# BloodAxe/segmentation-networks-benchmark

Measured on AMD Instinct MI355X. Metric: images/sec/GPU (fwd+bwd) ZF_UNET 224x224 bs=32; 1/2/4/8-GPU scaling, higher is better.
Workload: dtype bf16; 1 GPU; ZF_UNET 224x224 bf16 bs=32/GPU, bce_dice, SGD lr 1e-3, Dropout2d 0.2, train step torch_train.py:180-190 (configs[1]); global_batch=32, parallelism=dp1

## Files before the change

### segmentation-networks-benchmark_amd/csrc/common.h

```cpp
#pragma once
#include <hip/hip_runtime.h>
#include <hip/hip_ext.h>
#include <limits.h>
#include <stdint.h>
#include <stdio.h>
#include <string.h>

#include "../../include/segnb_hip.h"

typedef __attribute__((ext_vector_type(8))) __bf16 bf16x8_t;
typedef __attribute__((ext_vector_type(16))) float f32x16_t;

struct bf16_t {
    unsigned short bits;
};

void segnb_set_error(const char* fmt, ...);

#define SEGNB_CHECK_ARG_AS(who, cond, msg)                           \
    do {                                                             \
        if (!(cond)) {                                               \
            segnb_set_error("%s: bad argument: %s", who, msg);       \
            return SEGNB_E_BADARG;                                   \
        }                                                            \
// ... 126 lines not shown
    const long long yb = segnb_nhwc_bytes((long long)g->N * g->Ho * g->Wo, bn->ld_y, g->Co, 2);
    if (!segnb_fits_desc(yb)) return false;
    a.bn_y = (const bf16_t*)bn->y;
    a.bn_y_bytes = (unsigned)yb;
    a.bn_ld = bn->ld_y;
    a.bn_coef = bn->coef;
    a.bn_sums = bn->sums;
    a.bn_act = bn->act;
    a.bn_slope = bn->slope;
    return true;
}
template <class Args>
__attribute__((always_inline)) inline void take_act_epilogue(Args& a, const segnb_act_epilogue* ep) {
    a.ep_act = ep != nullptr ? ep->act : -1;
    a.ep_coef = ep != nullptr ? ep->coef : nullptr;
    a.ep_slope = ep != nullptr ? ep->slope : 0.f;
}
int segnb_fprop_thin_try(segnb_try_outcome* did, const segnb_conv_geom* g, const void* in, const void* wpacked, void* out,
                         hipStream_t stream, const segnb_bn_reduce_epilogue* bn);
int segnb_fprop_thin_ok(const segnb_conv_geom* g);
int segnb_knob_fprop_upd();
int segnb_knob_fprop_drop();
int segnb_knob_fprop_mask();
int segnb_fprop_dma_actmask_ok(const segnb_conv_geom* g);
int segnb_fprop_roll_actmask_ok(const segnb_conv_geom* g);
int segnb_knob_fprop_mf16();
int segnb_knob_fprop_rw();
int segnb_knob_fprop_ksplit();
float* segnb_head_scratch(size_t bytes, hipStream_t stream);
void segnb_head_bwd_finish(const float* part, int gx, int gy, int K, int C, int CT, float* dw, float* db, hipStream_t stream);
int segnb_knob_pack_blocks();
int segnb_knob_fprop_roll();
int segnb_knob_wg_cu_pct();
int segnb_knob_conv_cus();
int segnb_fprop_dma_read_stamps(unsigned long long* host_dst);
int segnb_fprop_s1_try(segnb_try_outcome* did, const segnb_conv_geom* g, const void* in, const void* wpacked, const float* bias, int bias_n,
                       void* out, double* stats, hipStream_t stream, const float* drop = nullptr, int ld_drop = 0, int stats_ld = 0);
int segnb_fprop_dma_try(segnb_try_outcome* did, const segnb_conv_geom* g, const void* in, unsigned in_bytes, const void* wpacked,
                        unsigned w_bytes, const float* bias, int bias_n, void* out, double* stats,
                        hipStream_t stream, const segnb_act_epilogue* ep = nullptr, const segnb_upcat_src* uc = nullptr,
                        const segnb_bn_reduce_epilogue* bn = nullptr);
int segnb_fprop_rw_try(segnb_try_outcome* did, const segnb_conv_geom* g, const void* in, unsigned in_bytes, const void* wpacked,
                       unsigned w_bytes, const float* bias, int bias_n, void* out, double* stats,
                       hipStream_t stream, const segnb_bn_reduce_epilogue* bn = nullptr,
                       const segnb_act_epilogue* ep = nullptr, const segnb_upcat_src* uc = nullptr,
                       const segnb_upcat_src* upsum = nullptr);
// ... 190 lines not shown
```

### segmentation-networks-benchmark_amd/csrc/conv_igemm.hip

```cpp
#include <stdlib.h>

#include "device.h"

namespace {

constexpr int LDS_ROW = 144;
constexpr int NT = 256;

struct FpropArgs {
    segnb_conv_geom g = {};
    const void* in = nullptr;
    const void* w = nullptr;
    const float* bias = nullptr;
    int bias_n = 0;
    const float* ep_coef = nullptr;
    int ep_act = -1;
    float ep_slope = 0.f;
    void* out = nullptr;
    double* stats = nullptr;
    int M = 0, Ktot = 0, ksteps = 0, MT = 0, NTL = 0, GM = 0;
    unsigned in_bytes = 0, w_bytes = 0;
    const void* bn_y = nullptr;
    int bn_ld = 0;
    const float* bn_coef = nullptr;
// ... 1256 lines not shown
extern "C" int segnb_conv_wgrad_upcat(const segnb_conv_geom* g, int dtype, const void* in, const segnb_upcat_src* src,
                                      const void* dout, float* dwp, int nslab, segnb_stream_t stream) {
    SEGNB_PLAN_RECORD(segnb_conv_wgrad_upcat, g, dtype, in, src, dout, dwp, nslab, stream);
    const segnb_wgrad_target* tgt;
    if (int rc = take_wgrad_target(__func__, g, &tgt)) return rc;
    SEGNB_CHECK_ARG(in && src && src->u && dout && dwp, "NULL tensor");
    SEGNB_CHECK_ARG(upcat_geom_ok(g, dtype, src->Cu), "geometry not served (segnb_conv_upcat_ok)");
    SEGNB_CHECK_ARG(nslab == segnb_conv_wgrad_slabs(g, dtype), "nslab differs from segnb_conv_wgrad_slabs()");
    segnb_try_outcome did;
    if (int rc = segnb_wgrad_s1_try(&did, g, in, dout, dwp, nslab, (hipStream_t)stream, false, nullptr, src, tgt)) return rc;
    return finish_wgrad(__func__, did, g, dwp, nslab, tgt, false, (hipStream_t)stream);
}

static bool out_slice_fits(const segnb_conv_geom* g, int ld) {
    return segnb_fits_desc(segnb_nhwc_bytes((long long)g->N * g->Ho * g->Wo, ld, g->Co, 2));
}

static bool bnreduce_general(const segnb_conv_geom* g) { return g->Ci <= 24 && g->Co >= 32 && g->Co % 8 == 0; }

extern "C" int segnb_conv_fprop_bnreduce_ok(const segnb_conv_geom* g, int dtype) {
    if (g == nullptr || dtype != SEGNB_BF16 || check_geom(g) || !segnb_knob_bnreduce_fused()) return 0;
    if (!whole_output_3x3_s1(g) || g->Co % 8 != 0) return 0;
    if (bnreduce_general(g)) return 1;
    if (segnb_fprop_general_forced() || !segnb_knob_fprop_dma() || !segnb_knob_fprop_rw() || g->Wo < 12) return 0;
    for (int t = 0; t < 9; ++t)
        if (g->dh[t] < -1 || g->dh[t] > 1 || g->dw[t] < -1 || g->dw[t] > 1) return 0;
    if (g->Ci % 32 != 0 || g->Ci > 96 || g->Co > 64) return 0;
    if (g->Co > 32 && g->Ci > 32) return 0;
    return 1;
}

extern "C" int segnb_conv_fprop_bnreduce(const segnb_conv_geom* g, int dtype, const void* in, const void* wpacked,
                                         void* out, const segnb_bn_reduce_epilogue* ep, segnb_stream_t stream) {
    SEGNB_PLAN_RECORD(segnb_conv_fprop_bnreduce, g, dtype, in, wpacked, out, ep, stream);
    if (int rc = check_geom(g)) return rc;
    SEGNB_CHECK_ARG(in && wpacked && out && ep && ep->y && ep->sums, "NULL argument");
    SEGNB_CHECK_ARG(ep->ld_y >= g->Co && ep->ld_y % 8 == 0, "bad y stride");
    unsigned inb, wb;
    if (int rc = conv_extents(__func__, g, 2, g->Ci, &inb, &wb)) return rc;
    const hipStream_t st = (hipStream_t)stream;
    int rc = 0;
    segnb_try_outcome did;
    if (ep->coef == nullptr) {
        SEGNB_CHECK_ARG(segnb_conv_fprop_actmask_ok(g, dtype), "geometry not served by a fused kernel (segnb_conv_fprop_actmask_ok)");
        if (segnb_fprop_roll_actmask_ok(g))
            rc = segnb_fprop_roll_try(&did, g, in, inb, wpacked, wb, nullptr, 0, out, nullptr, st, ep);
        else
            rc = segnb_fprop_dma_try(&did, g, in, inb, wpacked, wb, nullptr, 0, out, nullptr, st, nullptr, nullptr, ep);
    } else {
        SEGNB_CHECK_ARG(segnb_conv_fprop_bnreduce_ok(g, dtype), "geometry not served by a fused kernel (segnb_conv_fprop_bnreduce_ok)");
        if (bnreduce_general(g)) {
            SEGNB_CHECK_ARG(ep->ld_y % 8 == 0 && out_slice_fits(g, ep->ld_y), "bad y");
            return conv_fprop_impl(g, dtype, in, wpacked, nullptr, 0, out, nullptr, stream, nullptr, ep);
        }
        if (g->Ci <= 96) {
            rc = segnb_fprop_roll_try(&did, g, in, inb, wpacked, wb, nullptr, 0, out, nullptr, st, ep);
            if (!rc && !did) rc = segnb_fprop_rw_try(&did, g, in, inb, wpacked, wb, nullptr, 0, out, nullptr, st, ep);
        } else {
            rc = segnb_fprop_dma_try(&did, g, in, inb, wpacked, wb, nullptr, 0, out, nullptr, st, nullptr, nullptr, ep);
        }
    }
    return finish_fprop(__func__, rc, did, SEGNB_E_BADARG, "the fused kernel refused the launch");
}

extern "C" int segnb_conv_fprop_bnapply_ok(const segnb_conv_geom* g, int dtype) {
    if (g == nullptr || dtype != SEGNB_BF16 || check_geom(g) || !segnb_knob_bnreduce_fused()) return 0;
    if (!whole_output_3x3_s1(g) || g->Co % 8 != 0 || g->Co <= 32) return 0;
    return bnreduce_general(g) ? 1 : 0;
}

extern "C" int segnb_conv_fprop_bnsums(const segnb_conv_geom* g, int dtype, const void* in, const void* wpacked,
                                       const segnb_bn_reduce_epilogue* ep, segnb_stream_t stream) {
    SEGNB_PLAN_RECORD(segnb_conv_fprop_bnsums, g, dtype, in, wpacked, ep, stream);
    if (int rc = check_geom(g)) return rc;
    SEGNB_CHECK_ARG(in && wpacked && ep && ep->y && ep->coef && ep->sums, "NULL argument");
    SEGNB_CHECK_ARG(segnb_conv_fprop_bnapply_ok(g, dtype), "geometry not served (segnb_conv_fprop_bnapply_ok)");
    SEGNB_CHECK_ARG(ep->ld_y >= g->Co && ep->ld_y % 8 == 0 && out_slice_fits(g, ep->ld_y), "bad y");
    return conv_fprop_impl(g, dtype, in, wpacked, nullptr, 0, nullptr, nullptr, stream, nullptr, ep, nullptr, 1);
// ... 132 lines not shown
```

### segmentation-networks-benchmark_amd/csrc/fprop_dma.hip

```cpp
#include "common.h"

#include "fprop_dma.h"
#include "tile_div.h"

#include <mutex>
#include <vector>

namespace {

struct WsArgs : FdArgs {
    TileDiv div_hw, div_w;
};

__device__ unsigned long long g_stamps[3 * 256 * 4];
#define FD_STAMP(role, step, k)                                                                      \
    do {                                                                                            \
        if (DBG && ((a.dbg & 32) || ((a.dbg & 64) && (role) == 0 && (k) == 0)) && blockIdx.x == 0 && lane == 0 &&  \
            (step) < 256)                                                                            \
            g_stamps[((role) * 256 + (step)) * 4 + (k)] = __builtin_amdgcn_s_memtime();             \
    } while (0)

template <int BN_, int R_, int WT_, int CW_M_, bool TALL_ = false, bool MF16_ = true, int NTAP_ = 9, int UP_ = 0>
struct WsCfg {
    static constexpr bool UPD_ = UP_ == 1;
// ... 39 lines not shown
    static constexpr int OFF_BIAS = OFF_PIX + 4 * BM * 4;
    static constexpr int OFF_SCALE = OFF_BIAS + BN * 4;
    static constexpr int OFF_TICKET = OFF_SCALE + BN * 4;
    static constexpr int SMEM = OFF_TICKET + 16;
    static constexpr int RED_BYTES = MT * 16 * 8;
    static_assert(WM % (MF16_ ? 16 : 32) == 0 && WN % (MF16_ ? 16 : 32) == 0 && WAVES_M * WAVES_N == NCW, "wave tiling");
    static_assert(BPIECES % NBW == 0 && NBW + NAW == NLW, "fetch wave roles");
    static_assert(MT % OC == 0 && MT >= 2 * BN && RPT <= 8 && BM <= MT && BM % (MT / OC) == 0, "store pass / statistics threads");
    static constexpr bool MASK_OK = MF16_ && !TALL_ && BM == 256 && CW_M_ == 4 && SMEM + 2048 <= 160 * 1024;
    static_assert(RED_BYTES <= OFF_STG, "statistics reduction scratch");
    static_assert(SMEM <= 160 * 1024, "LDS");
    static_assert(TM + TN <= 6, "fragment wait statement");
};

template <class C_>
struct WsEpi : C_ {
    static constexpr bool EPI = true;
};
template <class C, class = void>
struct ws_epi_of : std::false_type {};
template <class C>
struct ws_epi_of<C, std::enable_if_t<C::EPI>> : std::true_type {};

template <class C, bool DBG, bool EP = false, bool STATS = true, bool SPLITK = false, bool MASK = false>
__global__ __launch_bounds__(512) void conv_fprop_ws_kernel(const WsArgs a) {
    static_assert(!SPLITK || (!EP && !DBG && C::UP == 0 && C::NTAP == 9), "split K: plain 3 x 3 forward / data gradient");
    static_assert(!MASK || (STATS && !EP && !DBG && !SPLITK && C::MF16 && C::UP == 0 && C::NTAP == 9 && !C::TALL && C::BM == 256 &&
                            C::BN == 64 && C::WAVES_M == 4 && C::SMEM + 2048 <= 160 * 1024),
                  "activation mask: plain 3 x 3 data gradient, 16x16x32 form, 256 x 64 tiles, 2 KB of mask bytes behind the LDS layout");
    constexpr int BN = C::BN, R = C::R, WT = C::WT, BM = C::BM, TM = C::TM, TN = C::TN, XC = C::XC;
    constexpr int NT = C::NT, NB = C::NB, APW = C::APW, APS = C::APS, BPW = C::BPW, OC = C::OC, NLW = C::NLW;
    constexpr int OUT_ROW = C::OUT_ROW, NF = TM + TN;
    constexpr int NTAP = C::NTAP, KW = C::KW;
    constexpr int SM = NTAP & 3;
    constexpr bool EPI = ws_epi_of<C>::value;
    static_assert(!EPI || (C::MF16 && !SPLITK && !EP && C::UP == 0 && C::NTAP == 9), "store rows on peeled taps: 16x16x32 form, 3 x 3 window, whole-K tiles");

    extern __shared__ __attribute__((aligned(1024))) unsigned char smem[];
    int* sPix = reinterpret_cast<int*>(smem + C::OFF_PIX);
    float* sBias = reinterpret_cast<float*>(smem + C::OFF_BIAS);
    const unsigned lds0 = (unsigned)(size_t)smem;

    const int tid = threadIdx.x, lane = tid & 63, wave = __builtin_amdgcn_readfirstlane(tid >> 6);
    const int r = lane & 31, h = lane >> 5;
    const bool loader = wave >= C::NCW;
    const int lw = wave - C::NCW;
    const int wm = (wave & 3) / C::WAVES_N, wn = (wave & 3) % C::WAVES_N;

    int L_ = xcd_remap(blockIdx.x, gridDim.x);
    int ks_ = 0, nt_, gq_;
    if (C::TALL && a.ntmajor) {
        gq_ = L_ % a.GM;
        L_ /= a.GM;
        if constexpr (SPLITK) {
            ks_ = L_ % a.KS;
            L_ /= a.KS;
        }
        nt_ = L_;
    } else {
// ... 72 lines not shown
                        const int pa_ = 2 * c, pb_ = 2 * c + 1;
                        const int ta = (2 * (t >> 1) - (pa_ >> 1) + 1) * 4 + (2 * (t & 1) - (pa_ & 1) + 1);
                        const int tb = (2 * (t >> 1) - (pb_ >> 1) + 1) * 4 + (2 * (t & 1) - (pb_ & 1) + 1);
        #pragma unroll
                        for (int pb = 0; pb < BPW; ++pb) {
                            const unsigned off = (unsigned)(((b_sec >> pb & 1u) ? tb : ta) * 32) * 2u;
                            dma16(lds0 + C::OFF_B + stage * C::B_STAGE + ((lw & 1) * BPW + pb) * 1024, b_voff[pb] + off, rs_w, 0u);
                        }
                        return;
                    }
                    const int pl = c / a.NCHP, sl = c - pl * a.NCHP;
                    const int t16 = (2 * (t >> 1) - (pl >> 1) + 1) * 4 + (2 * (t & 1) - (pl & 1) + 1);
                    soff = (unsigned)(t16 * a.Ci + sl * 64) * 2u;
                } else if constexpr (C::UPF) {
                    soff = (unsigned)((3 - t) * a.Ci + c * 64) * 2u;
                } else {
                    soff = (unsigned)(t * a.Ci + (c + c_off) * 64) * 2u;
                }
        #pragma unroll
                for (int pb = 0; pb < BPW; ++pb)
                    dma16(lds0 + C::OFF_B + stage * C::B_STAGE + ((lw & 1) * BPW + pb) * 1024, b_voff[pb], rs_w, soff);
            };

            fetch_b(0, 0, 0);
            fetch_b(0, 1, 1);
            fetch_b(0, 2, 2);
            asm volatile("s_waitcnt vmcnt(0)" ::: "memory");
            lds_barrier();
            for (; it < a.IT; it += a.GM) {
                for (int c = 0; c < a.NCH; ++c, ++cg) {
                    const int cn = c + 1 == a.NCH ? 0 : c + 1;
                    static_for<NTAP>([&](auto t_c) {
                        constexpr int t = decltype(t_c)::value;
                        constexpr int tf = t + 3 < NTAP ? t + 3 : t + 3 - NTAP;
                        const int cf = t + 3 < NTAP ? c : cn;
                        if (lw == 0) FD_STAMP(1, cg * 9 + t, 0);
                        if (!(DBG && (a.dbg & 1))) fetch_b(cf, tf, (cg * SM + t + 3) & (NB - 1));
                        if (lw == 0) FD_STAMP(1, cg * 9 + t, 1);
                        asm volatile("s_waitcnt vmcnt(%0)" ::"n"(BPW) : "memory");
                        if (lw == 0) FD_STAMP(1, cg * 9 + t, 2);
                        raw_barrier();
                        if (lw == 0) FD_STAMP(1, cg * 9 + t, 3);
                    });
                }
            }
        } else {
            unsigned a_rel[APW], a_xy[APW], a_voff[C::NPL][APW];
            unsigned a_uoff[APW];
            constexpr bool VCAT = !C::UPD && !C::UPF && !C::TALL;
            static_assert(!VCAT || (R % 2 == 0 && WT % 2 == 0), "virtual concat: even tile origins");
            unsigned a_urel[VCAT ? APW : 1];
            unsigned a_sec = 0;
            static_assert(APW <= 32, "one bit per halo piece");
            const bool vcat = VCAT && a.u != nullptr;
        #pragma unroll
            for (int pa = 0; pa < APW; ++pa) {
                const int pix = ((lw & 1) + C::NAW * pa) * 8 + (lane >> 3);
                const int q = lane & 7;
                const int xr = pix / XC, xc = pix - xr * XC;
                const int key = C::XC % 2 == 0 ? xc : pix;
                a_rel[pa] = (unsigned)((xr * a.Wi + xc) * (C::UPD ? 2 : 1)) * (unsigned)a.ld_x * 2u +
                            (unsigned)((q ^ ((key >> 1) & 7)) * 16);
                if constexpr (C::UPD)
                    if (a.P32)
                        a_rel[pa] = (unsigned)((xr * a.Wi + xc) * 2) * (unsigned)a.ld_x * 2u + (unsigned)(((q ^ ((key >> 1) & 7)) & 3) * 16);
                a_xy[pa] = pix < C::NPIX ? (unsigned)xr | ((unsigned)xc << 16) : 0x7fff7fffu;
                asm volatile("" : "+v"(a_xy[pa]));
                a_sec |= (unsigned)(((q ^ ((xc >> 1) & 7)) >> 2) & 1) << pa;
                if constexpr (VCAT)
                    a_urel[pa] = vcat ? (unsigned)(((a.dhmin + xr) >> 1) * a.Wu + ((a.dwmin + xc) >> 1)) * (unsigned)a.ld_u * 2u +
                                            (unsigned)((q ^ ((key >> 1) & 7)) * 16)
                                      : 0u;
// ... 129 lines not shown
                    }
                }
                auto go = [&](auto pl_c) {
                    constexpr int PL = decltype(pl_c)::value;
        #pragma unroll
                    for (int pa = 0; pa < APW; ++pa) {
                        if (pa >= p0 && pa < p1) {
                            const int piece = (lw & 1) + C::NAW * pa;
                            const unsigned dst = piece < C::APIECES ? lds0 + buf * C::A_BYTES + piece * 1024 : lds0 + C::OFF_DUMMY;
                            dma16(dst, a_voff[PL][pa], rs_x, soff);
                        }
                    }
                };
                if constexpr (C::UPD) {
                    if (pl == 0) go(std::integral_constant<int, 0>{});
                    else if (pl == 1) go(std::integral_constant<int, 1>{});
                    else if (pl == 2) go(std::integral_constant<int, 2>{});
                    else go(std::integral_constant<int, 3>{});
                } else {
                    go(std::integral_constant<int, 0>{});
                }
            };
            u32x4_t mreg[MASK ? 16 : 1];
            const __amdgpu_buffer_rsrc_t rs_y = make_rsrc(MASK ? a.bn_y : a.x, MASK ? a.bn_y_bytes : 0);
            auto mask_request = [&](int table) {
                const int t128 = (lw & 1) * 64 + lane;
                const int ch = n_base + (t128 & 7) * 8;
#pragma unroll
                for (int k = 0; k < 16; ++k) {
                    const int opix = sPix[table * BM + (t128 >> 3) + 16 * k];
                    const unsigned voff = (opix >= 0 && ch < a.Co) ? (unsigned)opix * (unsigned)a.bn_ld * 2u + (unsigned)ch * 2u : OOB;
                    mreg[k] = __builtin_amdgcn_raw_buffer_load_b128(rs_y, (int)voff, 0, 0);
                }
            };
            auto mask_publish = [&]() {
                const int t128 = (lw & 1) * 64 + lane;
                unsigned char* const dst = smem + C::SMEM + (t128 >> 3) * 8 + (t128 & 7);
#pragma unroll
                for (int k = 0; k < 16; ++k) {
                    const u32x4_t v = mreg[k];
                    unsigned b = 0u;
                    b |= __uint_as_float(v.x << 16) > 0.f ? 1u : 0u;
                    b |= __uint_as_float(v.x & 0xffff0000u) > 0.f ? 2u : 0u;
                    b |= __uint_as_float(v.y << 16) > 0.f ? 4u : 0u;
                    b |= __uint_as_float(v.y & 0xffff0000u) > 0.f ? 8u : 0u;
                    b |= __uint_as_float(v.z << 16) > 0.f ? 16u : 0u;
                    b |= __uint_as_float(v.z & 0xffff0000u) > 0.f ? 32u : 0u;
                    b |= __uint_as_float(v.w << 16) > 0.f ? 64u : 0u;
                    b |= __uint_as_float(v.w & 0xffff0000u) > 0.f ? 128u : 0u;
                    dst[16 * k * 8] = (unsigned char)b;
                }
                asm volatile("s_waitcnt lgkmcnt(0)" ::: "memory");
            };
            set_fetch_tile(it, 0);
            fetch_a(0, APW, 0, 0);
            if (a.NCH == 1) set_fetch_tile(it + a.GM, 1);
            asm volatile("s_waitcnt vmcnt(0)" ::: "memory");
            lds_barrier();
            int tile_no = 0;
            for (; it < a.IT; it += a.GM, ++tile_no) {
                for (int c = 0; c < a.NCH; ++c, ++cg) {
                    const bool last = c + 1 == a.NCH;
                    const int cn = last ? 0 : c + 1;
                    const bool next_last = last ? a.NCH == 1 : c + 2 == a.NCH;
                    const int setup_it = last ? it + 2 * a.GM : it + a.GM;
                    const int setup_tab = (tile_no + (last ? 2 : 1)) & 3;
                    const int abuf = cg & 1;
                    static_for<NTAP>([&](auto t_c) {
                        constexpr int t = decltype(t_c)::value;
                        if (lw == C::NBW) FD_STAMP(2, cg * 9 + t, 0);
                        if constexpr (t < C::A_STEPS)
                            if (!(DBG && (a.dbg & 2))) fetch_a(t * APS, (t + 1) * APS, cn, abuf ^ 1);
                        if constexpr (MASK) {
                            if constexpr (t == 0)
                                if (c == 0) mask_request(tile_no & 3);
                            if constexpr (t == NTAP - 1)
                                if (last) mask_publish();
                        }
                        if constexpr (t == NTAP - 2)
                            if (next_last) set_fetch_tile(setup_it, setup_tab);
                        if (lw == C::NBW) FD_STAMP(2, cg * 9 + t, 1);
                        if constexpr (t == NTAP - 2) {
                            asm volatile("s_waitcnt vmcnt(0)" ::: "memory");
                        }
                        if (lw == C::NBW) FD_STAMP(2, cg * 9 + t, 2);
                        raw_barrier();
                        if (lw == C::NBW) FD_STAMP(2, cg * 9 + t, 3);
                    });
                }
            }
        }
        asm volatile("s_waitcnt vmcnt(0)" ::: "memory");
        if constexpr (SPLITK) {
            raw_barrier();
            raw_barrier();
        }
        raw_barrier();
        raw_barrier();
        raw_barrier();
    } else {
        constexpr bool MF16 = C::MF16;
        int tile_no_out = 0;
        bool pending_out = false;
        constexpr int TM16 = C::TM16, TN16 = C::TN16;
        int b_rd[MF16 ? 1 : TN];
        int a_rd[MF16 ? 1 : 9][MF16 ? 1 : TM];
// ... 700 lines not shown
    return ws_launch_form<C>(a, stream);
}

using WsCfg14 = WsCfg<64, 14, 14, 2, false, true>;

bool ws14_serves(const WsArgs& a) {
    return a.H % 14 == 0 && a.W % 14 == 0 && a.W <= 56 && a.Co > 32 && a.bn_y == nullptr && a.ep_act < 0 && !a.dbg &&
           a.up_out == nullptr && segnb_knob_fprop_mf16();
}

int launch_ws14(WsArgs& a, hipStream_t stream) {
    using C = WsCfg14;
    using CE = WsEpi<C>;
    static const int attr_rc = segnb_opt_in_lds("fprop_ws", C::SMEM, conv_fprop_ws_kernel<C, false>, conv_fprop_ws_kernel<C, false, false, false>,
                                                conv_fprop_ws_kernel<CE, false>, conv_fprop_ws_kernel<CE, false, false, false>);
    if (attr_rc) return attr_rc;
    if (!ws_tile_grid<C>(a, (a.Co + C::BN - 1) / C::BN)) return SEGNB_LAUNCH_DECLINED;
    a.NCH = a.Ci / 64;
    if (g_segnb_census_on) segnb_census("tile:ws14");
    if (ws_epi_selected(WS_EPI_DEFAULT)) return ws_launch_form<CE, true>(a, stream);
    return ws_launch_form<C, true>(a, stream);
}

template <class C>
int launch_ws_upd(WsArgs& a, hipStream_t stream) {
    static const int attr_rc = segnb_opt_in_lds("fprop_ws", C::SMEM, conv_fprop_ws_kernel<C, false, false, false>);
    if (attr_rc) return attr_rc;
    a.P32 = a.Ci == 32;
    a.NCHP = a.P32 ? 1 : a.Ci / 64;
    a.NCH = a.P32 ? 2 : 4 * a.NCHP;
    a.RPS = a.NCH * C::NTAP - 1 < C::RPT ? 2 : 1;
    if ((a.NCH * C::NTAP - 1) * a.RPS < C::RPT) return SEGNB_LAUNCH_DECLINED;
    if (!ws_tile_grid<C>(a, (a.Co + C::BN - 1) / C::BN)) return SEGNB_LAUNCH_DECLINED;
    hipLaunchKernelGGL((conv_fprop_ws_kernel<C, false, false, false>), dim3(a.GM * a.NTL), dim3(C::NT), C::SMEM, stream, a);
    return 0;
}

template <class C>
int launch_ws_upf(WsArgs& a, hipStream_t stream) {
    static const int attr_rc = segnb_opt_in_lds("fprop_ws", C::SMEM, conv_fprop_ws_kernel<C, false, false, true>);
    if (attr_rc) return attr_rc;
    a.NTLR = (a.Co + C::BN - 1) / C::BN;
    a.NCH = a.Ci / 64;
    a.NCHP = a.NCH;
    a.P32 = 0;
    a.RPS = a.NCH * C::NTAP - 1 < C::RPT ? 2 : 1;
// ... 14 lines not shown
int try_upd(const segnb_conv_geom* g, WsArgs& a, hipStream_t stream) {
    if (!upd_geometry(g)) return SEGNB_LAUNCH_DECLINED;
    a.Ktot = 16 * g->Ci;
    a.dhmin = a.dwmin = 0;
    for (int t = 0; t < 9; ++t) a.dh[t] = a.dw[t] = 0;
    a.dh[2] = a.dh[3] = 1;
    a.dw[1] = a.dw[3] = 1;
    const int gm = ws_blocks((g->Co + 63) / 64);
    const long long it0 = (long long)g->N * ((g->Ho + 7) / 8) * ((g->Wo + 31) / 32);
    const long long it1 = (long long)g->N * ((g->Ho + 15) / 16) * ((g->Wo + 15) / 16);
    int cfg = segnb_knob_fprop_dma_cfg();
    if (cfg < 0) cfg = (it0 + gm - 1) / gm < (it1 + gm - 1) / gm ? 0 : 1;
    if (cfg == 0) return launch_ws_upd<WsCfg<64, 8, 32, 4, false, true, 4, 1>>(a, stream);
    return launch_ws_upd<WsCfg<64, 16, 16, 4, false, true, 4, 1>>(a, stream);
}

constexpr unsigned WS14_DEFAULT_LEVELS = 7u;

int dispatch_fd(WsArgs& a, hipStream_t stream) {
    int cfg = segnb_knob_fprop_dma_cfg();
    bool row_major_taps = true;
    for (int t = 0; t < 9; ++t) row_major_taps = row_major_taps && a.dw[t] == a.dw[t % 3] && a.dh[t] == a.dh[3 * (t / 3)];
    const bool can14 = row_major_taps && ws14_serves(a);
    if (cfg == 3 && !can14) cfg = -1;
    if (cfg < 0) {
        if (a.Co <= 32) return SEGNB_LAUNCH_DECLINED;
        if (a.W <= 8) {
            if (a.W != 7 || a.H != 7) return SEGNB_LAUNCH_DECLINED;
            return launch_ws<WsCfg<64, 36, 7, 4, true, false>>(a, stream);
        }
        const int gm = ws_blocks((a.Co + 63) / 64);
        const long long it0 = (long long)a.N * ((a.H + 7) / 8) * ((a.W + 31) / 32);
        const long long it1 = (long long)a.N * ((a.H + 15) / 16) * ((a.W + 15) / 16);
        const long long r0 = (it0 + gm - 1) / gm, r1 = (it1 + gm - 1) / gm;
        cfg = r0 < r1 ? 0 : 1;
        if (a.bn_y != nullptr) cfg = 1;
        const bool same_stats = a.stats == nullptr || a.W == 14;
        if (can14 && same_stats && a.H == a.W && ((a.W == 14 && (WS14_DEFAULT_LEVELS & 1u)) || (a.W == 28 && (WS14_DEFAULT_LEVELS & 2u)) ||
                                                  (a.W == 56 && (WS14_DEFAULT_LEVELS & 4u)))) {
            const long long it3 = (long long)a.N * (a.H / 14) * (a.W / 14);
            const long long r3 = (it3 + gm - 1) / gm;
            if (r3 * WsCfg14::BM < (cfg == 0 ? r0 : r1) * 256) cfg = 3;
        }
    }
    if (cfg == 3) return launch_ws14(a, stream);
    if (segnb_knob_fprop_mf16() && row_major_taps) {
// ... 50 lines not shown
    const long long it0 = (long long)N * ((H + 7) / 8) * ((W + 31) / 32);
    const long long it1 = (long long)N * ((H + 15) / 16) * ((W + 15) / 16);
    int cfg = segnb_knob_fprop_dma_cfg();
    if (cfg < 0) cfg = (it0 + gm - 1) / gm < (it1 + gm - 1) / gm ? 0 : 1;
    const int rc = cfg == 0 ? launch_ws_upf<WsCfg<64, 8, 32, 4, false, true, 4, 2>>(a, stream)
                            : launch_ws_upf<WsCfg<64, 16, 16, 4, false, true, 4, 2>>(a, stream);
    return segnb_try_launched(did, rc);
}

int segnb_fprop_dma_actmask_ok(const segnb_conv_geom* g) {
    if (!segnb_knob_fprop_dma() || !segnb_knob_fprop_mask() || !segnb_knob_fprop_mf16() || segnb_knob_fprop_dma_cfg() == 2 ||
        segnb_fprop_general_forced())
        return 0;
    if (!whole_output_3x3_s1(g) || g->Ci % 64 != 0 || g->Co <= 32 || g->Co % 8 != 0 || g->Wo <= 8) return 0;
    for (int t = 0; t < 9; ++t)
        if (g->dh[t] != g->dh[3 * (t / 3)] || g->dw[t] != g->dw[t % 3]) return 0;
    if (!segnb_window_once_3x3(g, segnb_tap_window(g))) return 0;
    return segnb_fits_desc(segnb_nhwc_bytes((long long)g->N * g->Hi * g->Wi, g->ld_in, g->Ci, 2)) &&
                   segnb_fits_desc(segnb_nhwc_bytes((long long)g->N * g->Ho * g->Wo, g->ld_out, g->Co, 2))
               ? 1
               : 0;
}

extern "C" int segnb_conv_fprop_upd_ok(const segnb_conv_geom* g, int dtype) {
    if (g == nullptr || dtype != SEGNB_BF16) return 0;
    if (!segnb_knob_fprop_dma() || !segnb_knob_fprop_upd() || segnb_fprop_general_forced()) return 0;
    return upd_geometry(g) && segnb_fits_desc(segnb_nhwc_bytes((long long)g->N * g->Ho * g->Wo, g->ld_out, g->Co, 2)) ? 1 : 0;
}

int segnb_fprop_dma_read_stamps(unsigned long long* host_dst) {
    return (int)hipMemcpyFromSymbol(host_dst, HIP_SYMBOL(g_stamps), sizeof(unsigned long long) * 3 * 256 * 4);
}

int segnb_fprop_dma_try(segnb_try_outcome* did, const segnb_conv_geom* g, const void* in, unsigned in_bytes, const void* wpacked,
                        unsigned w_bytes, const float* bias, int bias_n, void* out, double* stats,
                        hipStream_t stream, const segnb_act_epilogue* ep, const segnb_upcat_src* uc,
                        const segnb_bn_reduce_epilogue* bn) {
    *did = SEGNB_TRY_DECLINED;
    if (!segnb_knob_fprop_dma()) return 0;
    if (bn != nullptr && (bn->coef != nullptr || bn->y == nullptr || bn->sums == nullptr || ep != nullptr || uc != nullptr ||
                          stats != nullptr || bias != nullptr || !segnb_taps_3x3(g) || !segnb_knob_fprop_mask()))
        return 0;
    if (g->ntaps == 16 && ep == nullptr && stats == nullptr && bias == nullptr && segnb_knob_fprop_upd()) {
        WsArgs a;
        a.x = (const bf16_t*)in;
        a.w = (const bf16_t*)wpacked;
        a.x_bytes = in_bytes;
        a.w_bytes = w_bytes;
        a.bias = nullptr;
        a.bias_n = 0;
        a.out = (bf16_t*)out;
        a.stats = nullptr;
        a.N = g->N; a.H = g->Ho; a.W = g->Wo; a.Hi = g->Hi; a.Wi = g->Wi;
        a.Ci = g->Ci; a.Co = g->Co; a.ld_x = g->ld_in; a.ld_out = g->ld_out;
        if (!segnb_fits_desc(segnb_nhwc_bytes((long long)g->N * g->Ho * g->Wo, g->ld_out, g->Co, 2), &a.out_bytes)) return 0;
        a.dbg = 0;
        a.u = nullptr;
        a.up_out = nullptr;
    a.no_prev = 0;
        a.bn_y = nullptr;
        a.ep_act = -1;
        a.ep_coef = nullptr;
        a.ep_slope = 0.f;
        const int rc = try_upd(g, a, stream);
// ... 10 lines not shown
    a.bias_n = bias_n;
    a.out = (bf16_t*)out;
    a.stats = stats;
    a.N = g->N; a.H = g->Ho; a.W = g->Wo; a.Hi = g->Hi; a.Wi = g->Wi;
    a.Ci = g->Ci; a.Co = g->Co; a.ld_x = g->ld_in; a.ld_out = g->ld_out;
    a.Ktot = 9 * g->Ci;
    if (!segnb_fits_desc(segnb_nhwc_bytes((long long)g->N * g->Ho * g->Wo, g->ld_out, g->Co, 2), &a.out_bytes)) return 0;
    a.dhmin = win.dhmin; a.dwmin = win.dwmin;
    segnb_rel_taps(g, win, a.dh, a.dw);
    a.dbg = segnb_knob_fprop_dma_dbg();
    a.up_out = nullptr;
    a.no_prev = 0;
    a.u = nullptr;
    if (uc != nullptr) {
        if (uc->Cu % 64 != 0 || uc->Cu <= 0 || uc->Cu >= g->Ci || (g->Hi & 1) || (g->Wi & 1) || g->Wo <= 8) return 0;
        a.u = (const bf16_t*)uc->u;
        a.ld_u = uc->ld_u;
        a.NCHU = uc->Cu / 64;
        a.Hu = g->Hi / 2;
        a.Wu = g->Wi / 2;
        if (!segnb_fits_desc(segnb_nhwc_bytes((long long)g->N * a.Hu * a.Wu, uc->ld_u, uc->Cu, 2), &a.u_bytes)) return 0;
    }
    a.bn_y = nullptr;
    a.bn_act = SEGNB_ACT_NONE;
    a.bn_slope = 0.f;
    if (bn != nullptr) {
        if (bn->ld_y % 8 != 0 || !take_bn_reduce(a, g, bn)) return 0;
        a.stats = bn->sums;
    }
    take_act_epilogue(a, ep);
    const int rc = dispatch_fd(a, stream);
    return segnb_try_launched(did, rc);
}
```

### segmentation-networks-benchmark_amd/csrc/runtime.hip

```cpp
#include <stdarg.h>
#include <stdlib.h>

#include "common.h"

static thread_local char g_err[512] = "";

void segnb_set_error(const char* fmt, ...) {
    va_list ap;
    va_start(ap, fmt);
    vsnprintf(g_err, sizeof(g_err), fmt, ap);
    va_end(ap);
}

int segnb_num_cus() {
    static int cus = 0;
    if (cus > 0) return cus;
    int dev = 0;
    hipDeviceProp_t prop;
    if (hipGetDevice(&dev) != hipSuccess || hipGetDeviceProperties(&prop, dev) != hipSuccess) return 256;
    cus = prop.multiProcessorCount > 0 ? prop.multiProcessorCount : 256;
    return cus;
}

extern "C" const char* segnb_last_error(void) { return g_err; }
// ... 278 lines not shown
    }
    return g_fprop_mask;
}
static int g_fprop_drop = -2;
int segnb_knob_fprop_drop() {
    if (g_fprop_drop == -2) {
        const char* e = getenv("SEGNB_FPROP_DROP");
        g_fprop_drop = (e != nullptr && e[0] == '0') ? 0 : 1;
    }
    return g_fprop_drop;
}
static int g_fprop_nostats = 1;
int segnb_knob_fprop_nostats() { return g_fprop_nostats; }
static int g_rw_store_waves = 4;
int segnb_knob_rw_store_waves() { return g_rw_store_waves; }
static int g_bnreduce_fused = -2;
int segnb_knob_bnreduce_fused() {
    if (g_bnreduce_fused == -2) {
        const char* e = getenv("SEGNB_BNREDUCE_FUSED");
        g_bnreduce_fused = (e != nullptr && e[0] == '0') ? 0 : 1;
    }
    return g_bnreduce_fused;
}
static int g_fprop_ksplit = -2;
int segnb_knob_fprop_ksplit() {
    if (g_fprop_ksplit == -2) {
        const char* e = getenv("SEGNB_FPROP_KSPLIT");
        g_fprop_ksplit = e != nullptr ? atoi(e) : 1;
    }
    return g_fprop_ksplit;
}
static int g_fprop_dma_dbg = 0;
int segnb_knob_fprop_dma_dbg() { return g_fprop_dma_dbg; }
static int g_fprop_dma_epi = -1;
int segnb_knob_fprop_dma_epi() { return g_fprop_dma_epi; }
extern "C" int segnb_wg_cu_share(int pct) {
    SEGNB_PLAN_RECORD(segnb_wg_cu_share, pct);
    g_wg_cu_pct = pct < 0 ? 0 : (pct > 100 ? 100 : pct);
    return 0;
}

static thread_local segnb_wgrad_target g_wg_target;
static thread_local bool g_wg_target_armed = false;
extern "C" int segnb_wgrad_target_arm(const segnb_wgrad_target* t) {
    SEGNB_PLAN_RECORD(segnb_wgrad_target_arm, t);
    SEGNB_CHECK_ARG(t != nullptr && t->gw != nullptr, "NULL target");
// ... 54 lines not shown
        g_wg_cu_pct = value < 0 ? 0 : (value > 100 ? 100 : value);
        return 0;
    }
    if (strcmp(key, "fprop_drop") == 0) {
        g_fprop_drop = value ? 1 : 0;
        return 0;
    }
    if (strcmp(key, "fprop_mask") == 0) {
        g_fprop_mask = value ? 1 : 0;
        return 0;
    }
    if (strcmp(key, "fprop_nostats") == 0) {
        g_fprop_nostats = value ? 1 : 0;
        return 0;
    }
    if (strcmp(key, "rw_store_waves") == 0) {
        g_rw_store_waves = value == 2 ? 2 : (value == 8 ? 8 : 4);
        return 0;
    }
    if (strcmp(key, "bnreduce_fused") == 0) {
        g_bnreduce_fused = value ? 1 : 0;
        return 0;
    }
    if (strcmp(key, "fprop_deepk") == 0) {
        g_fprop_deepk = value ? 1 : 0;
        return 0;
    }
    if (strcmp(key, "fprop_thin") == 0) {
        g_fprop_thin = value ? 1 : 0;
        return 0;
    }
    if (strcmp(key, "fprop_mf16") == 0) {
        g_fprop_mf16 = value ? 1 : 0;
        return 0;
    }
    if (strcmp(key, "call_census") == 0) {
        g_segnb_census_on = value ? 1 : 0;
        return 0;
    }
    if (strcmp(key, "fprop_ksplit") == 0) {
        g_fprop_ksplit = value < 0 ? 0 : value;
        return 0;
    }
    if (strcmp(key, "fprop_dma_epi") == 0) {
        g_fprop_dma_epi = value < 0 ? -1 : (value ? 1 : 0);
        return 0;
// ... 14 lines not shown
```

Measured before the change: 7003 images/s.

## Fuse BatchNorm-backward reductions into warp-specialized 14x14 data-gradient conv kernel

Adds a BNRED variant of the warp-specialized 14x14 fprop/dgrad kernel. It loads the saved BN input tile into extra LDS, recomputes the activation mask, and accumulates the per-channel BN-backward sums (sum of dy and sum of dy*xhat) in the conv epilogue. The sums are reduced through LDS in double precision and added with atomics into replicated buffers. This replaces the roll/rw kernels or a separate reduction pass for Ci%64==0, Co>32 layers up to 56x56 (112 with knob=2), removing an extra read of the gradient and y tensors. The cost is more LDS per block, which may lower occupancy, plus extra ALU work interleaved in the tap loop.

```diff
diff --git a/segmentation-networks-benchmark_amd/csrc/common.h b/segmentation-networks-benchmark_amd/csrc/common.h
--- a/segmentation-networks-benchmark_amd/csrc/common.h
+++ b/segmentation-networks-benchmark_amd/csrc/common.h
@@ -172,6 +172,8 @@
 int segnb_knob_fprop_upd();
 int segnb_knob_fprop_drop();
 int segnb_knob_fprop_mask();
+int segnb_knob_ws_bnreduce();
+int segnb_fprop_dma_bnreduce_ok(const segnb_conv_geom* g);
 int segnb_fprop_dma_actmask_ok(const segnb_conv_geom* g);
 int segnb_fprop_roll_actmask_ok(const segnb_conv_geom* g);
 int segnb_knob_fprop_mf16();
diff --git a/segmentation-networks-benchmark_amd/csrc/conv_igemm.hip b/segmentation-networks-benchmark_amd/csrc/conv_igemm.hip
--- a/segmentation-networks-benchmark_amd/csrc/conv_igemm.hip
+++ b/segmentation-networks-benchmark_amd/csrc/conv_igemm.hip
@@ -1302,6 +1302,7 @@
     if (g == nullptr || dtype != SEGNB_BF16 || check_geom(g) || !segnb_knob_bnreduce_fused()) return 0;
     if (!whole_output_3x3_s1(g) || g->Co % 8 != 0) return 0;
     if (bnreduce_general(g)) return 1;
+    if (segnb_fprop_dma_bnreduce_ok(g)) return 1;
     if (segnb_fprop_general_forced() || !segnb_knob_fprop_dma() || !segnb_knob_fprop_rw() || g->Wo < 12) return 0;
     for (int t = 0; t < 9; ++t)
         if (g->dh[t] < -1 || g->dh[t] > 1 || g->dw[t] < -1 || g->dw[t] > 1) return 0;
@@ -1333,7 +1334,7 @@
             SEGNB_CHECK_ARG(ep->ld_y % 8 == 0 && out_slice_fits(g, ep->ld_y), "bad y");
             return conv_fprop_impl(g, dtype, in, wpacked, nullptr, 0, out, nullptr, stream, nullptr, ep);
         }
-        if (g->Ci <= 96) {
+        if (g->Ci <= 96 && !segnb_fprop_dma_bnreduce_ok(g)) {
             rc = segnb_fprop_roll_try(&did, g, in, inb, wpacked, wb, nullptr, 0, out, nullptr, st, ep);
             if (!rc && !did) rc = segnb_fprop_rw_try(&did, g, in, inb, wpacked, wb, nullptr, 0, out, nullptr, st, ep);
         } else {
diff --git a/segmentation-networks-benchmark_amd/csrc/fprop_dma.hip b/segmentation-networks-benchmark_amd/csrc/fprop_dma.hip
--- a/segmentation-networks-benchmark_amd/csrc/fprop_dma.hip
+++ b/segmentation-networks-benchmark_amd/csrc/fprop_dma.hip
@@ -85,6 +85,20 @@
 template <class C>
 struct ws_epi_of<C, std::enable_if_t<C::EPI>> : std::true_type {};
 
+template <class C_>
+struct WsBnRed : C_ {
+    static constexpr bool BNRED = true;
+    static constexpr int BNY_BYTES = C_::R * C_::WT * 128;
+    static constexpr int OFF_BNY = C_::SMEM;
+    static constexpr int SMEM_BN = OFF_BNY + BNY_BYTES;
+    static_assert(C_::SMEM == 135696 && SMEM_BN == 160784 && SMEM_BN <= 160 * 1024, "LDS: layout + one y tile");
+    static_assert(OFF_BNY % 16 == 0, "16-byte pieces");
+};
+template <class C, class = void>
+struct ws_bnred_of : std::false_type {};
+template <class C>
+struct ws_bnred_of<C, std::enable_if_t<C::BNRED>> : std::true_type {};
+
 template <class C, bool DBG, bool EP = false, bool STATS = true, bool SPLITK = false, bool MASK = false>
 __global__ __launch_bounds__(512) void conv_fprop_ws_kernel(const WsArgs a) {
     static_assert(!SPLITK || (!EP && !DBG && C::UP == 0 && C::NTAP == 9), "split K: plain 3 x 3 forward / data gradient");
@@ -98,6 +112,10 @@
     constexpr int SM = NTAP & 3;
     constexpr bool EPI = ws_epi_of<C>::value;
     static_assert(!EPI || (C::MF16 && !SPLITK && !EP && C::UP == 0 && C::NTAP == 9), "store rows on peeled taps: 16x16x32 form, 3 x 3 window, whole-K tiles");
+    constexpr bool BNRED = ws_bnred_of<C>::value;
+    static_assert(!BNRED || (!STATS && !EP && !DBG && !SPLITK && !MASK && C::MF16 && C::UP == 0 && C::NTAP == 9 && !C::TALL && C::R == 14 &&
+                             C::WT == 14 && C::BN == 64),
+                  "BatchNorm-backward sums: plain 3 x 3 data gradient on 14 x 14 tiles");
 
     extern __shared__ __attribute__((aligned(1024))) unsigned char smem[];
     int* sPix = reinterpret_cast<int*>(smem + C::OFF_PIX);
@@ -216,6 +234,44 @@
                     dma16(lds0 + C::OFF_B + stage * C::B_STAGE + ((lw & 1) * BPW + pb) * 1024, b_voff[pb], rs_w, soff);
             };
 
+            constexpr int NYR_W = (R * WT + 15) / 16;
+            segnb_f32x2_t ws1[4], ws2[4], bn_sc[4], bn_sh[4], bn_mu[4];
+#pragma unroll
+            for (int w = 0; w < 4; ++w) ws1[w] = ws2[w] = segnb_f32x2_t{0.f, 0.f};
+            if constexpr (BNRED) {
+                const int ch = n_base + (((lw & 1) * 64 + lane) & 7) * 8;
+                const bool ok = ch < a.Co;
+                const float* const cf = a.bn_coef + (ok ? ch : 0);
+                const float on = ok ? 1.f : 0.f;
+#pragma unroll
+                for (int w = 0; w < 4; ++w) {
+                    bn_sc[w] = segnb_f32x2_t{cf[2 * w], cf[2 * w + 1]} * on;
+                    bn_sh[w] = segnb_f32x2_t{cf[a.Co + 2 * w], cf[a.Co + 2 * w + 1]} * on;
+                    bn_mu[w] = segnb_f32x2_t{cf[2 * a.Co + 2 * w], cf[2 * a.Co + 2 * w + 1]} * on;
+                }
+            }
+            auto bn_item = [&](int k) {
+                if constexpr (BNRED) {
+                    const int t128 = (lw & 1) * 64 + lane, ccw = t128 & 7;
+                    const int row = (t128 >> 3) + 16 * k;
+                    const bool live = (16 * k + 15 < R * WT || row < R * WT) && n_base + ccw * 8 < a.Co;
+                    const int rr = row < R * WT ? row : 0;
+                    const u32x4_t gq = *reinterpret_cast<const u32x4_t*>(smem + C::OFF_STG + rr * C::OUT_ROW + ccw * 16);
+                    const u32x4_t yq = *reinterpret_cast<const u32x4_t*>(smem + C::OFF_BNY + rr * 128 + ccw * 16);
+#pragma unroll
+                    for (int w = 0; w < 4; ++w) {
+                        const unsigned gw = live ? gq[w] : 0u, yw = yq[w];
+                        const segnb_f32x2_t g2 = {__uint_as_float(gw << 16), __uint_as_float(gw & 0xffff0000u)};
+                        const segnb_f32x2_t y2 = {__uint_as_float(yw << 16), __uint_as_float(yw & 0xffff0000u)};
+                        const segnb_f32x2_t z = (y2 - bn_mu[w]) * bn_sc[w] + bn_sh[w];
+                        const segnb_f32x2_t n2 = g2 * mask_neg;
+                        const unsigned pn = pack2bf(n2.x, n2.y);
+                        const segnb_f32x2_t d2 = {z.x > 0.f ? g2.x : __uint_as_float(pn << 16), z.y > 0.f ? g2.y : __uint_as_float(pn & 0xffff0000u)};
+                        ws1[w] += d2;
+                        ws2[w] += d2 * y2;
+                    }
+                }
+            };
             fetch_b(0, 0, 0);
             fetch_b(0, 1, 1);
             fetch_b(0, 2, 2);
@@ -230,6 +286,20 @@
                         const int cf = t + 3 < NTAP ? c : cn;
                         if (lw == 0) FD_STAMP(1, cg * 9 + t, 0);
                         if (!(DBG && (a.dbg & 1))) fetch_b(cf, tf, (cg * SM + t + 3) & (NB - 1));
+                        if constexpr (BNRED) {
+                            if (cg > c) {
+                                if (a.NCH == 1) {
+                                    if constexpr (t >= 1 && t <= 7) {
+                                        bn_item(2 * (t - 1));
+                                        if constexpr (2 * (t - 1) + 1 < NYR_W) bn_item(2 * (t - 1) + 1);
+                                    }
+                                } else if (c == 0) {
+                                    if constexpr (t >= 1) bn_item(t - 1);
+                                } else if (c == 1) {
+                                    if constexpr (t + 8 < NYR_W) bn_item(t + 8);
+                                }
+                            }
+                        }
                         if (lw == 0) FD_STAMP(1, cg * 9 + t, 1);
                         asm volatile("s_waitcnt vmcnt(%0)" ::"n"(BPW) : "memory");
                         if (lw == 0) FD_STAMP(1, cg * 9 + t, 2);
@@ -238,10 +308,45 @@
                     });
                 }
             }
+            if constexpr (BNRED) {
+                asm volatile("s_waitcnt vmcnt(0)" ::: "memory");
+                raw_barrier();
+                if (cg > 0) {
+#pragma unroll
+                    for (int k = 0; k < NYR_W; ++k) bn_item(k);
+                }
+                lds_barrier();
+                const int t128 = (lw & 1) * 64 + lane;
+                double* const red = reinterpret_cast<double*>(smem);
+#pragma unroll
+                for (int w = 0; w < 4; ++w) {
+                    red[t128 * 16 + 2 * w] = (double)ws1[w].x;
+                    red[t128 * 16 + 2 * w + 1] = (double)ws1[w].y;
+                    red[t128 * 16 + 8 + 2 * w] = (double)ws2[w].x;
+                    red[t128 * 16 + 8 + 2 * w + 1] = (double)ws2[w].y;
+                }
+                lds_barrier();
+                if (t128 < BN) {
+                    const int c8 = t128 >> 3, e = t128 & 7;
+                    double sum1 = 0.0, sum2 = 0.0;
+                    for (int j = 0; j < 16; ++j) {
+                        sum1 += red[(j * 8 + c8) * 16 + e];
+                        sum2 += red[(j * 8 + c8) * 16 + 8 + e];
+                    }
+                    const int co = n_base + t128;
+                    if (co < a.Co) {
+                        const double mu = (double)a.bn_coef[2 * a.Co + co], is = (double)a.bn_coef[3 * a.Co + co];
+                        double* const rep = a.bn_sums + (long long)(blockIdx.x % SEGNB_STAT_REPLICAS) * 2 * a.Co;
+                        atomicAdd(&rep[co], sum1);
+                        atomicAdd(&rep[a.Co + co], (sum2 - mu * sum1) * is);
+                    }
+                }
+                return;
+            }
         } else {
             unsigned a_rel[APW], a_xy[APW], a_voff[C::NPL][APW];
             unsigned a_uoff[APW];
-            constexpr bool VCAT = !C::UPD && !C::UPF && !C::TALL;
+            constexpr bool VCAT = !C::UPD && !C::UPF && !C::TALL && !BNRED;
             static_assert(!VCAT || (R % 2 == 0 && WT % 2 == 0), "virtual concat: even tile origins");
             unsigned a_urel[VCAT ? APW : 1];
             unsigned a_sec = 0;
@@ -417,7 +522,7 @@
                 }
             };
             u32x4_t mreg[MASK ? 16 : 1];
-            const __amdgpu_buffer_rsrc_t rs_y = make_rsrc(MASK ? a.bn_y : a.x, MASK ? a.bn_y_bytes : 0);
+            const __amdgpu_buffer_rsrc_t rs_y = make_rsrc((MASK || BNRED) ? a.bn_y : a.x, (MASK || BNRED) ? a.bn_y_bytes : 0);
             auto mask_request = [&](int table) {
                 const int t128 = (lw & 1) * 64 + lane;
                 const int ch = n_base + (t128 & 7) * 8;
@@ -444,6 +549,31 @@
                     b |= __uint_as_float(v.w << 16) > 0.f ? 64u : 0u;
                     b |= __uint_as_float(v.w & 0xffff0000u) > 0.f ? 128u : 0u;
                     dst[16 * k * 8] = (unsigned char)b;
+                }
+                asm volatile("s_waitcnt lgkmcnt(0)" ::: "memory");
+            };
+            constexpr int NYR = (R * WT + 15) / 16;
+            u32x4_t yreg[NYR];
+            auto bn_request = [&](int table) {
+                const int t128 = (lw & 1) * 64 + lane;
+                const int ch = n_base + (t128 & 7) * 8;
+#pragma unroll
+                for (int k = 0; k < NYR; ++k) {
+                    const int opix = sPix[table * BM + (t128 >> 3) + 16 * k];
+                    const unsigned voff = (opix >= 0 && ch < a.Co) ? (unsigned)opix * (unsigned)a.bn_ld * 2u + (unsigned)ch * 2u : OOB;
+                    yreg[k] = __builtin_amdgcn_raw_buffer_load_b128(rs_y, (int)voff, 0, 0);
+                }
+            };
+            auto bn_publish = [&]() {
+                const int t128 = (lw & 1) * 64 + lane;
+#pragma unroll
+                for (int k = 0; k < NYR; ++k) {
+                    const int row = (t128 >> 3) + 16 * k;
+                    if (16 * k + 15 < R * WT || row < R * WT) {
+                        if constexpr (BNRED) {
+                            *reinterpret_cast<u32x4_t*>(smem + C::OFF_BNY + row * 128 + (t128 & 7) * 16) = yreg[k];
+                        }
+                    }
                 }
                 asm volatile("s_waitcnt lgkmcnt(0)" ::: "memory");
             };
@@ -472,11 +602,19 @@
                             if constexpr (t == NTAP - 1)
                                 if (last) mask_publish();
                         }
+                        if constexpr (BNRED) {
+                            if constexpr (t == 0)
+                                if (c == 0) bn_request(tile_no & 3);
+                        }
                         if constexpr (t == NTAP - 2)
                             if (next_last) set_fetch_tile(setup_it, setup_tab);
                         if (lw == C::NBW) FD_STAMP(2, cg * 9 + t, 1);
                         if constexpr (t == NTAP - 2) {
                             asm volatile("s_waitcnt vmcnt(0)" ::: "memory");
+                        }
+                        if constexpr (BNRED) {
+                            if constexpr (t == NTAP - 1)
+                                if (last) bn_publish();
                         }
                         if (lw == C::NBW) FD_STAMP(2, cg * 9 + t, 2);
                         raw_barrier();
@@ -1223,6 +1361,34 @@
     return ws_launch_form<C, true>(a, stream);
 }
 
+int ws_bnred_max_side() { return segnb_knob_ws_bnreduce() >= 2 ? 112 : 56; }
+bool ws_bnred_gate(int H, int W) {
+    const int side = ws_bnred_max_side();
+    return segnb_knob_ws_bnreduce() != 0 && H % 14 == 0 && W % 14 == 0 && H <= side && W <= side;
+}
+bool ws14_bnred_serves(const WsArgs& a) {
+    return a.bn_y != nullptr && a.bn_coef != nullptr && a.bn_sums != nullptr && ws_bnred_gate(a.H, a.W) && a.Co > 32 && a.Co % 8 == 0 &&
+           a.bn_ld % 8 == 0 && a.stats == nullptr && a.bias == nullptr && a.u == nullptr && a.ep_act < 0 && !a.dbg && a.up_out == nullptr &&
+           segnb_knob_fprop_mf16();
+}
+
+int launch_ws14_bnred(WsArgs& a, hipStream_t stream) {
+    using CB = WsBnRed<WsCfg14>;
+    using CBE = WsEpi<CB>;
+    static const int attr_rc =
+        segnb_opt_in_lds("fprop_ws", CB::SMEM_BN, conv_fprop_ws_kernel<CB, false, false, false>, conv_fprop_ws_kernel<CBE, false, false, false>);
+    if (attr_rc) return attr_rc;
+    if (!ws_tile_grid<CB>(a, (a.Co + CB::BN - 1) / CB::BN)) return SEGNB_LAUNCH_DECLINED;
+    a.NCH = a.Ci / 64;
+    if (g_segnb_census_on) segnb_census("tile:ws14");
+    const dim3 grid(a.GM * a.NTL), block(CB::NT);
+    if (ws_epi_selected(WS_EPI_DEFAULT))
+        hipLaunchKernelGGL((conv_fprop_ws_kernel<CBE, false, false, false>), grid, block, CB::SMEM_BN, stream, a);
+    else
+        hipLaunchKernelGGL((conv_fprop_ws_kernel<CB, false, false, false>), grid, block, CB::SMEM_BN, stream, a);
+    return 0;
+}
+
 template <class C>
 int launch_ws_upd(WsArgs& a, hipStream_t stream) {
     static const int attr_rc = segnb_opt_in_lds("fprop_ws", C::SMEM, conv_fprop_ws_kernel<C, false, false, false>);
@@ -1283,6 +1449,10 @@
     bool row_major_taps = true;
     for (int t = 0; t < 9; ++t) row_major_taps = row_major_taps && a.dw[t] == a.dw[t % 3] && a.dh[t] == a.dh[3 * (t / 3)];
     const bool can14 = row_major_taps && ws14_serves(a);
+    if (a.bn_y != nullptr && a.bn_coef != nullptr) {
+        if ((cfg >= 0 && cfg != 3) || !row_major_taps || !ws14_bnred_serves(a)) return SEGNB_LAUNCH_DECLINED;
+        return launch_ws14_bnred(a, stream);
+    }
     if (cfg == 3 && !can14) cfg = -1;
     if (cfg < 0) {
         if (a.Co <= 32) return SEGNB_LAUNCH_DECLINED;
@@ -1379,6 +1549,22 @@
                : 0;
 }
 
+int segnb_fprop_dma_bnreduce_ok(const segnb_conv_geom* g) {
+    if (!segnb_knob_fprop_dma() || !segnb_knob_fprop_mf16() || segnb_knob_fprop_dma_dbg() || segnb_fprop_general_forced()) return 0;
+    const int cfg = segnb_knob_fprop_dma_cfg();
+    if (cfg >= 0 && cfg != 3) return 0;
+    if (!whole_output_3x3_s1(g) || g->Ci % 64 != 0 || g->Co <= 32 || g->Co % 8 != 0 || !ws_bnred_gate(g->Ho, g->Wo)) return 0;
+    if (g->Hi != g->Ho || g->Wi != g->Wo) return 0;
+    for (int t = 0; t < 9; ++t)
+        if (g->dh[t] != g->dh[3 * (t / 3)] || g->dw[t] != g->dw[t % 3]) return 0;
+    if (!segnb_window_once_3x3(g, segnb_tap_window(g))) return 0;
+    if ((long long)g->N * (g->Ho / 14) * (g->Wo / 14) + 2ll * segnb_knob_conv_cus() > (long long)TILE_DIV_MAX) return 0;
+    return segnb_fits_desc(segnb_nhwc_bytes((long long)g->N * g->Hi * g->Wi, g->ld_in, g->Ci, 2)) &&
+                   segnb_fits_desc(segnb_nhwc_bytes((long long)g->N * g->Ho * g->Wo, g->ld_out, g->Co, 2))
+               ? 1
+               : 0;
+}
+
 extern "C" int segnb_conv_fprop_upd_ok(const segnb_conv_geom* g, int dtype) {
     if (g == nullptr || dtype != SEGNB_BF16) return 0;
     if (!segnb_knob_fprop_dma() || !segnb_knob_fprop_upd() || segnb_fprop_general_forced()) return 0;
@@ -1395,8 +1581,8 @@
                         const segnb_bn_reduce_epilogue* bn) {
     *did = SEGNB_TRY_DECLINED;
     if (!segnb_knob_fprop_dma()) return 0;
-    if (bn != nullptr && (bn->coef != nullptr || bn->y == nullptr || bn->sums == nullptr || ep != nullptr || uc != nullptr ||
-                          stats != nullptr || bias != nullptr || !segnb_taps_3x3(g) || !segnb_knob_fprop_mask()))
+    if (bn != nullptr && (bn->y == nullptr || bn->sums == nullptr || ep != nullptr || uc != nullptr || stats != nullptr || bias != nullptr ||
+                          !segnb_taps_3x3(g) || (bn->coef == nullptr ? !segnb_knob_fprop_mask() : !segnb_fprop_dma_bnreduce_ok(g))))
         return 0;
     if (g->ntaps == 16 && ep == nullptr && stats == nullptr && bias == nullptr && segnb_knob_fprop_upd()) {
         WsArgs a;
@@ -1453,11 +1639,13 @@
         if (!segnb_fits_desc(segnb_nhwc_bytes((long long)g->N * a.Hu * a.Wu, uc->ld_u, uc->Cu, 2), &a.u_bytes)) return 0;
     }
     a.bn_y = nullptr;
+    a.bn_coef = nullptr;
+    a.bn_sums = nullptr;
     a.bn_act = SEGNB_ACT_NONE;
     a.bn_slope = 0.f;
     if (bn != nullptr) {
         if (bn->ld_y % 8 != 0 || !take_bn_reduce(a, g, bn)) return 0;
-        a.stats = bn->sums;
+        if (bn->coef == nullptr) a.stats = bn->sums;
     }
     take_act_epilogue(a, ep);
     const int rc = dispatch_fd(a, stream);
diff --git a/segmentation-networks-benchmark_amd/csrc/runtime.hip b/segmentation-networks-benchmark_amd/csrc/runtime.hip
--- a/segmentation-networks-benchmark_amd/csrc/runtime.hip
+++ b/segmentation-networks-benchmark_amd/csrc/runtime.hip
@@ -324,6 +324,14 @@
     }
     return g_bnreduce_fused;
 }
+static int g_ws_bnreduce = -2;
+int segnb_knob_ws_bnreduce() {
+    if (g_ws_bnreduce == -2) {
+        const char* e = getenv("SEGNB_WS_BNREDUCE");
+        g_ws_bnreduce = e == nullptr ? 1 : (e[0] == '0' ? 0 : (e[0] == '2' ? 2 : 1));
+    }
+    return g_ws_bnreduce;
+}
 static int g_fprop_ksplit = -2;
 int segnb_knob_fprop_ksplit() {
     if (g_fprop_ksplit == -2) {
@@ -424,6 +432,10 @@
         g_bnreduce_fused = value ? 1 : 0;
         return 0;
     }
+    if (strcmp(key, "ws_bnreduce") == 0) {
+        g_ws_bnreduce = value <= 0 ? 0 : (value >= 2 ? 2 : 1);
+        return 0;
+    }
     if (strcmp(key, "fprop_deepk") == 0) {
         g_fprop_deepk = value ? 1 : 0;
         return 0;
```

After: 7005 images/s, median of 5. No clear change (+0.0%).
